# maduc238/simple_distributed_machine_learning

Measured on AMD Instinct MI355X. Metric: samples/sec (whole node), 2-stage MLP on MNIST-shape synthetic, higher is better.
Workload: dtype fp32

## Files before the change

### simple_distributed_machine_learning_amd/csrc/kernels/head_block.h

```cpp
#pragma once

#include <hip/hip_runtime.h>

#include "head_tile.h"
#include "lds_dma.h"

namespace sdml {
namespace hblk {

typedef float hb_f32x16 __attribute__((ext_vector_type(16)));
typedef float hb_f32x4 __attribute__((ext_vector_type(4)));
typedef _Float16 hb_f16x8 __attribute__((ext_vector_type(8)));
typedef _Float16 hb_f16x4 __attribute__((ext_vector_type(4)));
typedef short hb_s16x4 __attribute__((ext_vector_type(4)));
typedef float hb_f32x2 __attribute__((ext_vector_type(2)));
typedef _Float16 hb_f16x2 __attribute__((ext_vector_type(2)));
typedef unsigned hb_u32x2 __attribute__((ext_vector_type(2)));

constexpr int ROWS = 256, HID = 128, NW = 8, NT = 512;
constexpr int PLANE_B = HID * ROWS * 2;
constexpr int DLT_OFF = 2 * PLANE_B;
constexpr int DLT_PLANE_B = 16 * ROWS * 2;
constexpr int RED_OFF = DLT_OFF + 2 * DLT_PLANE_B;
constexpr int RED_FLOATS = 168;
// ... 59 lines not shown
  hb_f32x4 w2c;
  headtile::f32x4m b;
  int tg[2];
};
template <int C>
__device__ __forceinline__ void load_operands(const Args& a, int m0, int M, int wave, int lane, Operands& o) {
  const int r = lane & 15, g = lane >> 4;
  o.w2c = reinterpret_cast<const hb_f32x4*>(a.w2)[min(wave * 64 + lane, C * HID / 4 - 1)];
#pragma unroll
  for (int v = 0; v < 4; ++v) o.b[v] = a.b2[min(4 * g + v, C - 1)];
#pragma unroll
  for (int it = 0; it < 2; ++it)
    o.tg[it] = reinterpret_cast<const int*>(a.target)[2 * (size_t)min(m0 + 16 * (wave + NW * it) + r, M - 1)];
}

struct NoOp {
  __device__ void operator()() const {}
};
template <int C, class Prep, class Hook, class PostB1 = NoOp>
__device__ __forceinline__ void block_head(Prep&& prep, unsigned char* smem, const Args& a, const Operands& ops, int m0,
                                           int M, int wave, int lane, Hook&& hook, long long* stamp,
                                           PostB1&& post_b1 = PostB1{}) {
  static_assert(C >= 2 && C <= 16 && C % 2 == 0, "one 16-class tile; dl stored by class pairs");
  auto st = [&](int k) {
    if (stamp && lane == 0) stamp[k] = (long long)__builtin_amdgcn_s_memtime();
  };
  float* red = reinterpret_cast<float*>(smem + RED_OFF);
  const int wm = wave & 3, wn = wave >> 2, h2 = lane >> 5, r32 = lane & 31;
  const int r = lane & 15, g = lane >> 4;
  const int tid = wave * 64 + lane;
  headtile::f32x4m bv;
#pragma unroll
  for (int v = 0; v < 4; ++v) bv[v] = (4 * g + v) < C ? ops.b[v] : 0.f;
  const int tg[2] = {ops.tg[0], ops.tg[1]};

  hb_f32x16 y[2][2];
  prep(y);
  float hm = 0.f;
#pragma unroll
  for (int i = 0; i < 2; ++i)
#pragma unroll
    for (int j = 0; j < 2; ++j)
#pragma unroll
      for (int q = 0; q < 16; ++q) hm = fmaxf(hm, fabsf(y[i][j][q]));
  hm = wv::max64(hm);
  const float wc = fmaxf(fmaxf(fabsf(ops.w2c[0]), fabsf(ops.w2c[1])), fmaxf(fabsf(ops.w2c[2]), fabsf(ops.w2c[3])));
  const float wmw = wv::max64(wc);
  if (lane == 0) {
    red[wave] = hm;
    red[160 + wave] = wmw;
  }
  __syncthreads();
  st(17);
  post_b1();
  float bm = red[0], wm2 = red[160];
#pragma unroll
  for (int w = 1; w < NW; ++w) {
    bm = fmaxf(bm, red[w]);
    wm2 = fmaxf(wm2, red[160 + w]);
// ... 1 lines not shown
  const int Eh = bexp(bm), Ew = bexp(wm2), Ed = bexp(a.loss_scale);
  const float sh = p2(14 - Eh), sw = p2(14 - Ew), sd = p2(14 - Ed);
  const hb_f32x2 sh2 = {sh, sh}, sd2 = {sd, sd};
  {
    const bool ok = tid < C * HID / 4;
    const hb_f32x2 sw2 = {sw, sw};
    const hb_f32x2 x01 = hb_f32x2{ok ? ops.w2c[0] : 0.f, ok ? ops.w2c[1] : 0.f} * sw2;
    const hb_f32x2 x23 = hb_f32x2{ok ? ops.w2c[2] : 0.f, ok ? ops.w2c[3] : 0.f} * sw2;
    const hb_f16x2 h01 = __builtin_convertvector(x01, hb_f16x2), h23 = __builtin_convertvector(x23, hb_f16x2);
    const hb_f16x2 l01 = lo_pair(h01, x01), l23 = lo_pair(h23, x23);
    unsigned char* dst = smem + W2_OFF + (tid >> 5) * W2PP + 8 * (tid & 31);
    *reinterpret_cast<hb_f16x4*>(dst) = hb_f16x4{h01[0], h01[1], h23[0], h23[1]};
    *reinterpret_cast<hb_f16x4*>(dst + W2PL) = hb_f16x4{l01[0], l01[1], l23[0], l23[1]};
  }

  const int ib0 = hid_base(64 * wn + r32, 16 * wm + h2), ib1 = hid_base(64 * wn + 32 + r32, 16 * wm + h2);
#pragma unroll
  for (int i = 0; i < 2; ++i)
#pragma unroll
    for (int j = 0; j < 2; ++j) {
#pragma unroll
      for (int rq = 0; rq < 4; ++rq) {
        const hb_f32x2 x01 = hb_f32x2{y[i][j][4 * rq], y[i][j][4 * rq + 1]} * sh2;
        const hb_f32x2 x23 = hb_f32x2{y[i][j][4 * rq + 2], y[i][j][4 * rq + 3]} * sh2;
        const hb_f16x2 h01 = __builtin_convertvector(x01, hb_f16x2), h23 = __builtin_convertvector(x23, hb_f16x2);
        const hb_f16x4 hi = {h01[0], h01[1], h23[0], h23[1]};
        const hb_f16x2 l01 = lo_pair(h01, x01), l23 = lo_pair(h23, x23);
        const hb_f16x4 lo = {l01[0], l01[1], l23[0], l23[1]};
        const int o = (j ? ib1 : ib0) ^ (8 * (8 * i + 2 * rq));
        *reinterpret_cast<hb_f16x4*>(smem + o) = hi;
        *reinterpret_cast<hb_f16x4*>(smem + HPL + o) = lo;
      }
    }
  __syncthreads();
  st(18);
  hb_f16x8 wp[4][2];
#pragma unroll
  for (int kk = 0; kk < 4; ++kk)
#pragma unroll
    for (int p = 0; p < 2; ++p)
      wp[kk][p] = *reinterpret_cast<const hb_f16x8*>(smem + W2_OFF + p * W2PL + r * W2PP + 2 * (32 * kk + 8 * g));

  headtile::TileAcc acc;
  acc.zero();
  const float zsc = p2(Eh - 14) * p2(Ew - 14);
  hb_f32x4 dbs = {0.f, 0.f, 0.f, 0.f};
  const int lb0 = hoff(0, 8 * g + (r >> 2), 4 * wave + (r & 3)), lb1 = hoff(0, 8 * g + 4 + (r >> 2), 4 * wave + (r & 3));
  const __amdgpu_buffer_rsrc_t dlr = dma_rsrc(a.dl, (unsigned)((size_t)M * C * 4));
// ... 119 lines not shown
```

### simple_distributed_machine_learning_amd/csrc/kernels/mlp_u8.hip

```cpp
#include <hip/hip_runtime.h>

#include <algorithm>
#include <cstdlib>
#include <type_traits>

#include "head_block.h"
#include "head_reduce.h"
#include "head_tile.h"
#include "lds_dma.h"
#include "kernels.h"
#include "mma_prims.h"
#include "sgd_rule.h"
#include "wave_ops.h"
#include "u8_planes.h"

namespace sdml {
namespace {

typedef unsigned u32x4 __attribute__((ext_vector_type(4)));
typedef _Float16 f16x2 __attribute__((ext_vector_type(2)));

constexpr int FBN = 128;
constexpr int FBK = 64;
constexpr int NS = 2;
constexpr int NSUB = FBK / 16;
constexpr int NPL = kU8FwdPlanes;
constexpr int B_PLANE = FBN * FBK * 2;
constexpr int XCH = FBK / 16;
constexpr int WCH = FBK / 8;
static_assert(FBK == 32 || FBK == 64, "swizzles below are written for 32- and 64-deep K-steps");

template <int WMT, int NWR = 4, int NSG = NS>
struct Geo {
  static constexpr int THREADS = 128 * NWR;
  static constexpr int WAVES = THREADS / 64;
  static constexpr int BM = NWR * 32 * WMT;
  static constexpr int A_BYTES = BM * FBK;
  static constexpr int STAGE = A_BYTES + NPL * B_PLANE;
  static constexpr int GLDS_X = A_BYTES / 1024 / WAVES;
  static constexpr int GLDS_W = NPL * B_PLANE / 1024 / WAVES;
  static constexpr int GLDS_PER_STAGE = GLDS_X + GLDS_W;
  static_assert(GLDS_X * 1024 * WAVES == A_BYTES && GLDS_W * 1024 * WAVES == NPL * B_PLANE, "DMA split");
  static constexpr int EPR = WAVES * 64 * 64 * 4 <= 128 * 1024 ? 64 : 32;
  static constexpr int SMEM = std::max(NSG * STAGE, WAVES * EPR * 64 * 4);
  static_assert(SMEM <= 160 * 1024, "LDS");
};

__device__ __forceinline__ int xpos(int r, int c) { return c ^ (XCH == 2 ? (r >> 3) & 1 : (r >> 2) & 3); }
__device__ __forceinline__ int wpos(int r, int c) { return c ^ (WCH == 4 ? (r >> 2) & 3 : (r >> 1) & 7); }

template <int N>
__device__ __forceinline__ void wait_vmcnt() {
  asm volatile("s_waitcnt vmcnt(%0)" ::"n"(N) : "memory");
}

__device__ __forceinline__ f16x2 h2_of(unsigned v, unsigned sel) {
  const unsigned t = __builtin_amdgcn_perm(0x64646464u, v, sel);
  return __builtin_bit_cast(f16x2, t) - f16x2{(_Float16)1024.f, (_Float16)1024.f};
}
__device__ __forceinline__ f16x8 widen8h(unsigned lo, unsigned hi) {
  const f16x2 a = h2_of(lo, 0x04010400u), b = h2_of(lo, 0x04030402u);
  const f16x2 c = h2_of(hi, 0x04010400u), d = h2_of(hi, 0x04030402u);
  return f16x8{a[0], a[1], b[0], b[1], c[0], c[1], d[0], d[1]};
}

__device__ __forceinline__ f32x16 mfma(f16x8 a, f16x8 b, f32x16 c) {
  return __builtin_amdgcn_mfma_f32_32x32x16_f16(a, b, c, 0, 0, 0);
}

struct FwdParams {
  const unsigned char* X;
  const u16* Wp;
  const float* bias;
  float* C;
  int M, N, K, Kp, ldx, ldc;
  float scale;
  int relu;
  int prio;
  unsigned* mask;
  float* wmax;
  U8HeadArgs head;
  int pf_stride;
// ... 34 lines not shown
  constexpr int WROWS = 1024 / (2 * FBK);
  constexpr int WINST = FBN / WROWS;
  const size_t plane = (size_t)p.N * p.Kp;
#pragma unroll
  for (int u = 0; u < G::GLDS_W; ++u) {
    if (G::GLDS_X + u < U0 || G::GLDS_X + u >= U1) continue;
    const int q = wave + G::WAVES * u;
    const int pl = q / WINST;
    const int row = WROWS * (q % WINST) + lane / WCH;
    const int ch = wpos(row, lane % WCH);
    bdma16(rw, (unsigned)(2 * (pl * plane + (size_t)(n0 + row) * p.Kp + k0 + 8 * ch)), st + G::A_BYTES + 1024 * q);
  }
}

template <int C, int NWR>
__device__ __forceinline__ void fused_head_epilogue(const FwdParams& p, const f32x16 (&acc)[2][2], unsigned char* smem,
                                                    int m0, int wave, int lane, int wm, int wn,
                                                    const hblk::Operands& ops, const float (&bv1)[2], long long* stamp,
                                                    int hb);
template <int C>
__device__ __forceinline__ void fused_head_prefetch(const FwdParams& p, int m0, int wave, int lane, int wn,
                                                    hblk::Operands& ops, float (&bv1)[2]);

template <int MODE, int WMT, int TAIL, int NWR, int HEADC = 0, int NSK = NS, int DMAS = 0>
__global__ void __launch_bounds__(128 * NWR, NWR == 2 ? 2 : 1) u8_fwd_kernel(FwdParams p) {
  constexpr int NS = NSK;
  using G = Geo<WMT, NWR, NSK>;
  static_assert(HEADC == 0 || ((WMT == 2 || WMT == 4) && NWR == 4), "the fused head epilogue: 8 waves of 64 x 64");
  constexpr bool HALVES = HEADC > 0 && WMT == 4;
  auto tile_row = [](int i) { return HALVES ? 32 * (i & 1) + 256 * (i >> 1) : 32 * i; };
  static_assert(HEADC == 0 || G::SMEM <= hblk::LDS_BYTES, "the prefetch scratch KiB sits past the ring and the head");
  constexpr int STAGE = G::STAGE, GLDS_PER_STAGE = G::GLDS_PER_STAGE;
  constexpr int SMEM_BYTES = HEADC ? std::max(G::SMEM, hblk::LDS_BYTES) + 1024 : G::SMEM;
  __shared__ __attribute__((aligned(16))) unsigned char smem[SMEM_BYTES];
  const int m0 = blockIdx.x * G::BM, n0 = blockIdx.y * FBN;
  const int lane = threadIdx.x & 63;
  const int wave = __builtin_amdgcn_readfirstlane(threadIdx.x >> 6);
  const int wm = wave % NWR, wn = wave / NWR;
  if (p.prio && wave >= G::WAVES / 2) __builtin_amdgcn_s_setprio(1);
  const int h = lane >> 5, r32 = lane & 31;
  U8_STAMP(0, __builtin_amdgcn_s_memrealtime);
  U8_STAMP(1, __builtin_amdgcn_s_memtime);
  hblk::Operands hops;
  float hb1[2];

  f32x16 acc[WMT][2];
#pragma unroll
  for (int i = 0; i < WMT; ++i)
#pragma unroll
    for (int j = 0; j < 2; ++j) acc[i][j] = f32x16{};

  int aoff[XCH / 2], boff[NSUB];
  {
    const int row = (HALVES ? wm * 64 : wm * 32 * WMT) + r32;
#pragma unroll
    for (int c = 0; c < XCH / 2; ++c) aoff[c] = row * FBK + 16 * xpos(row, (XCH / 2) * h + c);
  }
  {
    const int row = wn * 64 + r32;
#pragma unroll
    for (int s = 0; s < NSUB; ++s) boff[s] = G::A_BYTES + row * (2 * FBK) + 16 * wpos(row, NSUB * h + s);
  }

  auto load_a = [&](const unsigned char* st, int s2, u32x4 (&ar)[WMT]) {
#pragma unroll
    for (int i = 0; i < WMT; ++i) {
      if constexpr (MODE == 3) ar[i] = u32x4{(unsigned)aoff[s2], 1u, 2u, 3u};
      else ar[i] = *reinterpret_cast<const u32x4*>(st + aoff[s2] + FBK * tile_row(i));
    }
  };
  auto load_b = [&](const unsigned char* st, int s, f16x8 (&b)[2][NPL]) {
#pragma unroll
    for (int j = 0; j < 2; ++j)
#pragma unroll
      for (int pl = 0; pl < NPL; ++pl) {
        if constexpr (MODE == 3) b[j][pl] = __builtin_bit_cast(f16x8, bf16x8{(short)boff[s], (short)pl, (short)j, 2, 3, 4, 5, 6});
        else b[j][pl] = *reinterpret_cast<const f16x8*>(st + boff[s] + 64 * FBK * j + pl * B_PLANE);
      }
  };
  auto compute = [&](int s, const u32x4 (&ar)[WMT], const f16x8 (&b)[2][NPL]) {
#pragma unroll
    for (int i = 0; i < WMT; ++i) {
      const u32x4 v = ar[i];
      f16x8 a;
      if constexpr (MODE == 5) a = __builtin_bit_cast(f16x8, v);
      else a = (s & 1) ? widen8h(v[2], v[3]) : widen8h(v[0], v[1]);
#pragma unroll
      for (int j = 0; j < 2; ++j)
#pragma unroll
        for (int pl = NPL - 1; pl >= 0; --pl) acc[i][j] = mfma(a, b[j][pl], acc[i][j]);
    }
  };
  constexpr int DMA_AT = MODE == 8 ? 0 : (MODE == 9 ? 1 : -1);
  static_assert(DMAS == 0 || (NSK == 2 && DMA_AT < 0 && MODE != 11 && GLDS_PER_STAGE == 6),
                "spread DMA: the 2-stage production loop, 6 pieces per wave");
  constexpr bool PIPE = MODE == 11;
  auto kstep = [&](const unsigned char* st, auto ns_c, auto&& dma, auto&& dma_part) {
    constexpr int NS_ = decltype(ns_c)::value;
    if constexpr (MODE == 1) return;
    if constexpr (PIPE) {
      u32x4 ar[2][WMT];
      f16x8 b[2][2][NPL];
      load_a(st, 0, ar[0]);
      load_b(st, 0, b[0]);
      dma();
#pragma unroll
      for (int s = 0; s < NS_; ++s) {
        if (s + 1 < NS_) {
          if ((s + 1) % 2 == 0) load_a(st, (s + 1) >> 1, ar[((s + 1) >> 1) & 1]);
          load_b(st, s + 1, b[(s + 1) & 1]);
        }
        __builtin_amdgcn_sched_barrier(0);
        compute(s, ar[(s >> 1) & 1], b[s & 1]);
        __builtin_amdgcn_sched_barrier(0);
      }
    } else if constexpr (DMAS == 2) {
      u32x4 ar[2][WMT];
      f16x8 b[2][2][NPL];
      load_a(st, 0, ar[0]);
      load_b(st, 0, b[0]);
#pragma unroll
      for (int s = 0; s < NS_; ++s) {
        if (s + 1 < NS_) {
          if ((s + 1) % 2 == 0) load_a(st, (s + 1) >> 1, ar[((s + 1) >> 1) & 1]);
          load_b(st, s + 1, b[(s + 1) & 1]);
        }
        compute(s, ar[(s >> 1) & 1], b[s & 1]);
        dma_part(s);
      }
    } else {
      u32x4 ar[WMT];
      f16x8 b[2][NPL];
#pragma unroll
      for (int s = 0; s < NS_; ++s) {
        if (s % 2 == 0) load_a(st, s >> 1, ar);
        load_b(st, s, b);
        compute(s, ar, b);
        if (s == DMA_AT) dma();
        if constexpr (DMAS == 1) dma_part(s);
      }
    }
  };

  const int nk = p.Kp / FBK;
#pragma unroll
  for (int t = 0; t < NS - 1; ++t)
    if (t < nk) issue_stage<WMT, NWR>(p, smem + t * STAGE, m0, n0, t * FBK, wave, lane);
  auto sync_step = [&](int t, auto issue_c) {
    const int ahead = min(NS - 2, nk - 1 - t);
    if constexpr (NS >= 4) {
      if (ahead >= 2) wait_vmcnt<2 * GLDS_PER_STAGE>();
      else if (ahead == 1) wait_vmcnt<GLDS_PER_STAGE>();
      else wait_vmcnt<0>();
    } else if constexpr (NS == 3) {
// ... 29 lines not shown
        },
        [&](int sub) {
          if (sub == 0) issue_stage<WMT, NWR, 0, 2>(p, nxt, m0, n0, k1, wave, lane);
          else if (sub == 1) issue_stage<WMT, NWR, 2, 4>(p, nxt, m0, n0, k1, wave, lane);
          else if (sub == 2) issue_stage<WMT, NWR, 4, 1 << 20>(p, nxt, m0, n0, k1, wave, lane);
        });
  }
  {
    sync_step(nk - 1, std::integral_constant<bool, (NS > 2)>{});
    kstep(smem + ((nk - 1) % NS) * STAGE, std::integral_constant<int, TAIL>{}, no_dma, no_dma_part);
  }
  U8_STAMP(15, __builtin_amdgcn_s_memtime);
  if constexpr (MODE == 10) {
    float keep = 0.f;
#pragma unroll
    for (int i = 0; i < WMT; ++i)
#pragma unroll
      for (int j = 0; j < 2; ++j)
#pragma unroll
        for (int r = 0; r < 16; ++r) keep += acc[i][j][r];
    if (keep == 12345.f && lane == 99) p.stamps[0] = 1;
    return;
  }

  if constexpr (HEADC > 0) {
    long long* stp = MODE == 7 ? p.stamps + ((size_t)blockIdx.x * G::WAVES + wave) * U8_NSTAMP : nullptr;
    if constexpr (!HALVES) {
      fused_head_epilogue<HEADC, NWR>(p, acc, smem, m0, wave, lane, wm, wn, hops, hb1, stp, (int)blockIdx.x);
    } else {
      typedef const f32x16 Half[2][2];
      fused_head_epilogue<HEADC, NWR>(p, *reinterpret_cast<Half*>(&acc[0][0]), smem, m0, wave, lane, wm, wn, hops, hb1,
                                      stp, 2 * (int)blockIdx.x);
      if (m0 + hblk::ROWS < p.M) {
        __syncthreads();
        fused_head_prefetch<HEADC>(p, m0 + hblk::ROWS, wave, lane, wn, hops, hb1);
        fused_head_epilogue<HEADC, NWR>(p, *reinterpret_cast<Half*>(&acc[2][0]), smem, m0 + hblk::ROWS, wave, lane, wm,
                                        wn, hops, hb1, nullptr, 2 * (int)blockIdx.x + 1);
      }
    }
    U8_STAMP(22, __builtin_amdgcn_s_memtime);
    U8_STAMP(U8_NSTAMP - 1, __builtin_amdgcn_s_memrealtime);
    return;
  }
  __syncthreads();
  constexpr int EPR = G::EPR, NI2 = EPR / 32;
  float* T = reinterpret_cast<float*>(smem) + wave * EPR * 64;
  float bv[2];
#pragma unroll
  for (int j = 0; j < 2; ++j) bv[j] = p.bias ? p.bias[n0 + wn * 64 + 32 * j + r32] : 0.f;
  float vmax = 0.f;
#pragma unroll
  for (int ip = 0; ip < WMT / NI2; ++ip) {
    asm volatile("s_waitcnt lgkmcnt(0)" ::: "memory");
#pragma unroll
    for (int j = 0; j < 2; ++j)
#pragma unroll
      for (int i2 = 0; i2 < NI2; ++i2)
#pragma unroll
        for (int r = 0; r < 16; ++r) {
          float y = acc[NI2 * ip + i2][j][r] * p.scale + bv[j];
          if (p.relu) y = fmaxf(y, 0.f);
          T[(32 * i2 + (r & 3) + 8 * (r >> 2) + 4 * h) * 64 + 32 * j + r32] = y;
        }
    asm volatile("s_waitcnt lgkmcnt(0)" ::: "memory");
    __builtin_amdgcn_wave_barrier();
#pragma unroll
    for (int q = 0; q < EPR / 4; ++q) {
      const int rr = 4 * q + (lane >> 4);
      const int row = m0 + wm * 32 * WMT + EPR * ip + rr;
      const f32x4 v = *reinterpret_cast<const f32x4*>(T + rr * 64 + 4 * (lane & 15));
      if constexpr (MODE == 6) {
        if (v[0] == 12345.f && row < 0) *reinterpret_cast<f32x4*>(p.C) = v;
      } else if (row < p.M) {
        *reinterpret_cast<f32x4*>(p.C + (size_t)row * p.ldc + n0 + wn * 64 + 4 * (lane & 15)) = v;
        vmax = fmaxf(fmaxf(vmax, fmaxf(fabsf(v[0]), fabsf(v[1]))), fmaxf(fabsf(v[2]), fabsf(v[3])));
      }
      if (p.mask) {
        unsigned w = ((v[0] > 0.f ? 1u : 0u) | (v[1] > 0.f ? 2u : 0u) | (v[2] > 0.f ? 4u : 0u) |
                      (v[3] > 0.f ? 8u : 0u)) << (4 * (lane & 7));
        w |= __shfl_xor(w, 1);
        w |= __shfl_xor(w, 2);
        w |= __shfl_xor(w, 4);
        if ((lane & 7) == 0 && row < p.M)
          p.mask[(size_t)row * (p.N / 32) + (n0 + wn * 64) / 32 + ((lane & 15) >> 3)] = w;
      }
    }
  }
  if (p.wmax) {
    for (int off = 32; off > 0; off >>= 1) vmax = fmaxf(vmax, __shfl_xor(vmax, off));
    if (lane == 0) p.wmax[((size_t)blockIdx.y * gridDim.x + blockIdx.x) * G::WAVES + wave] = vmax;
  }
}

template <int Q>
__device__ __forceinline__ void mask_words(const f32x16 (&y)[2][2], int (&mw)[2]) {
  if constexpr (Q < 64) {
    constexpr int i = Q >> 5, j = (Q >> 4) & 1, r = Q & 15, rw = 32 * i + 8 * (r >> 2);
    const unsigned long long b0 = __ballot(y[i][j][r] > 0.f), b1 = __ballot(y[i][j][r + 1] > 0.f);
    const unsigned long long b2 = __ballot(y[i][j][r + 2] > 0.f), b3 = __ballot(y[i][j][r + 3] > 0.f);
    asm("s_nop 4\n\t"
        "v_writelane_b32 %0, %1, %9\n\tv_writelane_b32 %0, %2, %10\n\t"
        "v_writelane_b32 %0, %3, %11\n\tv_writelane_b32 %0, %4, %12\n\t"
        "v_writelane_b32 %0, %5, %13\n\tv_writelane_b32 %0, %6, %14\n\t"
        "v_writelane_b32 %0, %7, %15\n\tv_writelane_b32 %0, %8, %16"
        : "+v"(mw[j])
        : "s"((unsigned)b0), "s"((unsigned)(b0 >> 32)), "s"((unsigned)b1), "s"((unsigned)(b1 >> 32)),
          "s"((unsigned)b2), "s"((unsigned)(b2 >> 32)), "s"((unsigned)b3), "s"((unsigned)(b3 >> 32)),
          "i"(rw), "i"(rw + 4), "i"(rw + 1), "i"(rw + 5), "i"(rw + 2), "i"(rw + 6), "i"(rw + 3), "i"(rw + 7));
    mask_words<Q + 4>(y, mw);
  }
}

template <int C>
__device__ __forceinline__ hblk::Args fused_head_args(const FwdParams& p, int hb) {
  const U8HeadArgs& hd = p.head;
  hblk::Args a;
  a.w2 = hd.w2;
  a.b2 = hd.b2;
  a.target = hd.target;
  a.loss_scale = hd.loss_scale;
  a.train = true;
  a.dl = hd.dl;
  a.part = hd.part + (size_t)hb * (C * 128 + C + 2);
  a.bound = hd.bound + hb;
  return a;
}

template <int C>
__device__ __forceinline__ void fused_head_prefetch(const FwdParams& p, int m0, int wave, int lane, int wn,
                                                    hblk::Operands& ops, float (&bv1)[2]) {
  hblk::load_operands<C>(fused_head_args<C>(p, 0), m0, p.M, wave, lane, ops);
#pragma unroll
  for (int j = 0; j < 2; ++j) bv1[j] = p.bias[wn * 64 + 32 * j + (lane & 31)];
}

template <int C, int NWR>
__device__ __forceinline__ void fused_head_epilogue(const FwdParams& p, const f32x16 (&acc)[2][2], unsigned char* smem,
                                                    int m0, int wave, int lane, int wm, int wn,
                                                    const hblk::Operands& ops, const float (&bv1)[2], long long* stamp,
                                                    int hb) {
  static_assert(NWR == 4, "head_block.h: 8 waves of 64 x 64, 256 rows");
  const U8HeadArgs& hd = p.head;
  const int h2 = lane >> 5;
  if (stamp && lane == 0) stamp[16] = (long long)__builtin_amdgcn_s_memtime();
  const hblk::Args a = fused_head_args<C>(p, hb);
  auto prep = [&](hblk::hb_f32x16 (&y)[2][2]) {
    const hblk::hb_f32x2 sc2 = {p.scale, p.scale};
#pragma unroll
    for (int i = 0; i < 2; ++i)
#pragma unroll
      for (int j = 0; j < 2; ++j) {
        const hblk::hb_f32x2 b2 = {bv1[j], bv1[j]};
#pragma unroll
        for (int r = 0; r < 16; r += 2) {
          const hblk::hb_f32x2 v = __builtin_elementwise_fma(hblk::hb_f32x2{acc[i][j][r], acc[i][j][r + 1]}, sc2, b2);
          y[i][j][r] = fmaxf(v[0], 0.f);
          y[i][j][r + 1] = fmaxf(v[1], 0.f);
        }
      }
    if (m0 + hblk::ROWS > p.M) {
#pragma unroll
      for (int i = 0; i < 2; ++i)
#pragma unroll
        for (int j = 0; j < 2; ++j)
#pragma unroll
          for (int r = 0; r < 16; ++r)
            if (m0 + wm * 64 + 32 * i + (r & 3) + 8 * (r >> 2) + 4 * h2 >= p.M) y[i][j][r] = 0.f;
    }
    int mw[2] = {0, 0};
    mask_words<0>(y, mw);
    const int row = m0 + wm * 64 + lane;
    if (row < p.M) *reinterpret_cast<uint2*>(hd.mask + (size_t)row * 4 + 2 * wn) = uint2{(unsigned)mw[0], (unsigned)mw[1]};
  };
  const bool pf = p.pf_stride > 0 && (int)blockIdx.x + p.pf_stride < (int)gridDim.x;
  auto post_b1 = [&]() {
    if (pf) {
      const int m1 = ((int)blockIdx.x + p.pf_stride) * hblk::ROWS;
      const dma_i32x4 rx = dma_rsrc4(p.X, (unsigned)((size_t)p.M * p.ldx));
#pragma unroll
      for (int u = 0; u < 2; ++u) {
        const int row = 16 * (wave + 8 * u) + (lane >> 2);
        const unsigned voff = (unsigned)((size_t)min(m1 + row, p.M - 1) * p.ldx + 16 * (lane & 3));
        bdma16_asm(rx, voff, 0u, smem + hblk::LDS_BYTES);
      }
    }
  };
  hblk::block_head<C>(prep, smem, a, ops, m0, p.M, wave, lane, [](int, int, bool, const float (&)[4]) {}, stamp,
                      post_b1);
  if (pf) asm volatile("s_waitcnt vmcnt(0)" ::: "memory");
}

__global__ void __launch_bounds__(256) split_planes_pad_kernel(const float* __restrict__ w, u16* __restrict__ out,
                                                               int N, int K, int Kp) {
  const int64_t i = (int64_t)blockIdx.x * 256 + threadIdx.x;
  const int64_t n = (int64_t)N * Kp;
  if (i >= n) return;
  const int r = (int)(i / Kp), k = (int)(i % Kp);
  const float x = k < K ? w[(size_t)r * K + k] : 0.f;
  u16 hi, lo;
  u8_fwd_planes_of(x, hi, lo);
  out[i] = hi;
  out[n + i] = lo;
}
// ... 854 lines not shown
  int dev = 0;
  if (hipGetDevice(&dev) != hipSuccess || dev < 0 || dev >= 64) return nullptr;
  if (!words[dev]) {
    hipStreamCaptureStatus cs = hipStreamCaptureStatusNone;
    if (hipStreamIsCapturing(stream, &cs) != hipSuccess || cs != hipStreamCaptureStatusNone) return nullptr;
    void* w = nullptr;
    if (hipMalloc(&w, 4096 * sizeof(unsigned)) != hipSuccess) return nullptr;
    if (hipMemset(w, 0, 4096 * sizeof(unsigned)) != hipSuccess) return nullptr;
    words[dev] = static_cast<unsigned*>(w);
  }
  return words[dev];
}

static int tail_substeps(int K) {
  const int v = K - ((K + FBK - 1) / FBK - 1) * FBK;
  if (v > FBK / 2 - 8) return NSUB;
  if (NSUB == 4 && v > 16) return 3;
  if (NSUB == 4 && v > 8) return 2;
  return 1;
}

int u8_fwd_kpad(int K) { return (K + FBK - 1) / FBK * FBK; }

bool u8_fwd_supported(int M, int N, int K, int ldx, const void* X) {
  return M >= 256 && N % FBN == 0 && K >= 16 && K % 16 == 0 && ldx % 16 == 0 &&
         (reinterpret_cast<uintptr_t>(X) & 15) == 0 && (int64_t)M * ldx < (int64_t(1) << 31);
}

bool u8_wgrad_supported(int M, int N, int K, int ldx, const void* X, const void* dz) {
  return K == GKC && N % GHN == 0 && M % GBK == 0 && M >= GBK && ldx % 16 == 0 &&
         (reinterpret_cast<uintptr_t>(X) & 15) == 0 && (reinterpret_cast<uintptr_t>(dz) & 15) == 0 &&
         (int64_t)M * ldx < (int64_t(1) << 31);
}

// ... 168 lines not shown
  }();
#else
  constexpr int mode = 0;
#endif
  bool w16;
  int wmt, bm;
  u8_fwd_geometry(M, w16, wmt, bm);
  const dim3 grid((M + bm - 1) / bm, N / FBN);
  const int tail = tail_substeps(K);
#define FWD_LAUNCH(MD, W, T, R) \
  hipLaunchKernelGGL((u8_fwd_kernel<MD, W, T, R>), grid, dim3(Geo<W, R>::THREADS), 0, stream, p)
#define FWD_TAILS(W, R)                          \
  do {                                           \
    switch (tail) {                              \
      case 1: FWD_LAUNCH(0, W, 1, R); break;     \
      case 2: FWD_LAUNCH(0, W, 2, R); break;     \
      case 3: FWD_LAUNCH(0, W, 3, R); break;     \
      default: FWD_LAUNCH(0, W, NSUB, R);        \
    }                                            \
  } while (0)
#define FWD_MODE(MD)                                \
  do {                                              \
    if (w16) FWD_LAUNCH(MD, 2, NSUB, 8);            \
    else if (wmt == 4) FWD_LAUNCH(MD, 4, NSUB, 4);  \
    else FWD_LAUNCH(MD, 2, NSUB, 4);                \
  } while (0)
#ifdef SDML_KERNEL_EXPERIMENTS
  if (mode == 1) FWD_MODE(1);
  else if (mode == 2) FWD_MODE(2);
  else if (mode == 3) FWD_MODE(3);
  else if (mode == 4) FWD_MODE(4);
  else if (mode == 5) FWD_MODE(5);
// ... 100 lines not shown
      case 4: FHM(4); break;
      case 5: FHM(5); break;
      case 8: FHM(8); break;
      case 9: FHM(9); break;
      case 10: FHM(10); break;
      case 11: FHM(11); break;
      default: abort();
    }
#undef FHM
    return;
  }
  if (g_u8_stamps && head.C == 10) {
    p.stamps = g_u8_stamps;
    switch (tail) {
      case 1: hipLaunchKernelGGL((u8_fwd_kernel<7, 2, 1, 4, 10>), grid, dim3(512), 0, stream, p); break;
      case 2: hipLaunchKernelGGL((u8_fwd_kernel<7, 2, 2, 4, 10>), grid, dim3(512), 0, stream, p); break;
      case 3: hipLaunchKernelGGL((u8_fwd_kernel<7, 2, 3, 4, 10>), grid, dim3(512), 0, stream, p); break;
      default: hipLaunchKernelGGL((u8_fwd_kernel<7, 2, NSUB, 4, 10>), grid, dim3(512), 0, stream, p);
    }
    return;
  }
#endif
  const dim3 grid512((M + Geo<4, 4>::BM - 1) / Geo<4, 4>::BM, 1);
  if (rows512) p.pf_stride = 0;
#define FH_LAUNCH(T, CC)                                                                                    \
  do {                                                                                                      \
    if (rows512) hipLaunchKernelGGL((u8_fwd_kernel<0, 4, T, 4, CC>), grid512, dim3(512), 0, stream, p);       \
    else if (spread == 2) hipLaunchKernelGGL((u8_fwd_kernel<0, 2, T, 4, CC, NS, 2>), grid, dim3(512), 0, stream, p); \
    else if (spread) hipLaunchKernelGGL((u8_fwd_kernel<0, 2, T, 4, CC, NS, 1>), grid, dim3(512), 0, stream, p); \
    else hipLaunchKernelGGL((u8_fwd_kernel<0, 2, T, 4, CC>), grid, dim3(512), 0, stream, p);               \
  } while (0)
#define FH_LAUNCH3(T) hipLaunchKernelGGL((u8_fwd_kernel<0, 2, T, 4, 10, 3>), grid, dim3(512), 0, stream, p)
#define FH_TAILS(CC)                      \
  do {                                    \
    switch (tail) {                       \
      case 1: FH_LAUNCH(1, CC); break;    \
      case 2: FH_LAUNCH(2, CC); break;    \
      case 3: FH_LAUNCH(3, CC); break;    \
      default: FH_LAUNCH(NSUB, CC);       \
    }                                     \
  } while (0)
  if (head.C == 10 && knob(KNOB_U8_FH_STAGES) == 3) {
    switch (tail) {
      case 1: FH_LAUNCH3(1); break;
      case 2: FH_LAUNCH3(2); break;
      case 3: FH_LAUNCH3(3); break;
      default: FH_LAUNCH3(NSUB);
    }
    return;
  }
  switch (head.C) {
    case 10: FH_TAILS(10); break;
    case 2: FH_TAILS(2); break;
    case 16: FH_TAILS(16); break;
    default: abort();
  }
#undef FH_TAILS
#undef FH_LAUNCH3
#undef FH_LAUNCH
}

// ... 2 lines not shown
```

Baseline: 993.5 million.

## Switch u8 forward GEMM from 32x32x16 to 16x16x32 MFMA tiles

Replaces the 32x32x16 f16 MFMA in the u8 forward kernel with the 16x16x32 variant. This reworks the accumulator layout (4x4 tiles of f32x4), the A/B LDS swizzles, the load/widen/compute pipeline, the tail sub-step logic and the epilogue. The fused head path gets a Map16 lane mapping and a rewritten ReLU mask packing to match the new accumulator layout. The aim is a shorter MFMA latency and better operand reuse per K-step. The cost is more LDS B loads per column tile and a reworked, riskier swizzle and mask mapping.

```diff
diff --git a/simple_distributed_machine_learning_amd/csrc/kernels/head_block.h b/simple_distributed_machine_learning_amd/csrc/kernels/head_block.h
--- a/simple_distributed_machine_learning_amd/csrc/kernels/head_block.h
+++ b/simple_distributed_machine_learning_amd/csrc/kernels/head_block.h
@@ -1,6 +1,8 @@
 #pragma once
 
 #include <hip/hip_runtime.h>
+
+#include <type_traits>
 
 #include "head_tile.h"
 #include "lds_dma.h"
@@ -97,13 +99,18 @@
     o.tg[it] = reinterpret_cast<const int*>(a.target)[2 * (size_t)min(m0 + 16 * (wave + NW * it) + r, M - 1)];
 }
 
+struct Map32 {};
+struct Map16 {};
+
 struct NoOp {
   __device__ void operator()() const {}
 };
-template <int C, class Prep, class Hook, class PostB1 = NoOp>
+template <int C, class Prep, class Hook, class PostB1 = NoOp, class Map = Map32>
 __device__ __forceinline__ void block_head(Prep&& prep, unsigned char* smem, const Args& a, const Operands& ops, int m0,
                                            int M, int wave, int lane, Hook&& hook, long long* stamp,
-                                           PostB1&& post_b1 = PostB1{}) {
+                                           PostB1&& post_b1 = PostB1{}, Map = Map{}) {
+  constexpr bool M16 = std::is_same<Map, Map16>::value;
+  constexpr int YA = M16 ? 4 : 2, YV = M16 ? 4 : 16;
   static_assert(C >= 2 && C <= 16 && C % 2 == 0, "one 16-class tile; dl stored by class pairs");
   auto st = [&](int k) {
     if (stamp && lane == 0) stamp[k] = (long long)__builtin_amdgcn_s_memtime();
@@ -117,15 +124,15 @@
   for (int v = 0; v < 4; ++v) bv[v] = (4 * g + v) < C ? ops.b[v] : 0.f;
   const int tg[2] = {ops.tg[0], ops.tg[1]};
 
-  hb_f32x16 y[2][2];
+  typename std::conditional<M16, hb_f32x4, hb_f32x16>::type y[YA][YA];
   prep(y);
   float hm = 0.f;
 #pragma unroll
-  for (int i = 0; i < 2; ++i)
-#pragma unroll
-    for (int j = 0; j < 2; ++j)
-#pragma unroll
-      for (int q = 0; q < 16; ++q) hm = fmaxf(hm, fabsf(y[i][j][q]));
+  for (int i = 0; i < YA; ++i)
+#pragma unroll
+    for (int j = 0; j < YA; ++j)
+#pragma unroll
+      for (int q = 0; q < YV; ++q) hm = fmaxf(hm, fabsf(y[i][j][q]));
   hm = wv::max64(hm);
   const float wc = fmaxf(fmaxf(fabsf(ops.w2c[0]), fabsf(ops.w2c[1])), fmaxf(fabsf(ops.w2c[2]), fabsf(ops.w2c[3])));
   const float wmw = wv::max64(wc);
@@ -157,24 +164,36 @@
     *reinterpret_cast<hb_f16x4*>(dst + W2PL) = hb_f16x4{l01[0], l01[1], l23[0], l23[1]};
   }
 
-  const int ib0 = hid_base(64 * wn + r32, 16 * wm + h2), ib1 = hid_base(64 * wn + 32 + r32, 16 * wm + h2);
-#pragma unroll
-  for (int i = 0; i < 2; ++i)
-#pragma unroll
-    for (int j = 0; j < 2; ++j) {
-#pragma unroll
-      for (int rq = 0; rq < 4; ++rq) {
-        const hb_f32x2 x01 = hb_f32x2{y[i][j][4 * rq], y[i][j][4 * rq + 1]} * sh2;
-        const hb_f32x2 x23 = hb_f32x2{y[i][j][4 * rq + 2], y[i][j][4 * rq + 3]} * sh2;
-        const hb_f16x2 h01 = __builtin_convertvector(x01, hb_f16x2), h23 = __builtin_convertvector(x23, hb_f16x2);
-        const hb_f16x4 hi = {h01[0], h01[1], h23[0], h23[1]};
-        const hb_f16x2 l01 = lo_pair(h01, x01), l23 = lo_pair(h23, x23);
-        const hb_f16x4 lo = {l01[0], l01[1], l23[0], l23[1]};
-        const int o = (j ? ib1 : ib0) ^ (8 * (8 * i + 2 * rq));
-        *reinterpret_cast<hb_f16x4*>(smem + o) = hi;
-        *reinterpret_cast<hb_f16x4*>(smem + HPL + o) = lo;
+  auto put = [&](float v0, float v1, float v2, float v3, int o) {
+    const hb_f32x2 x01 = hb_f32x2{v0, v1} * sh2;
+    const hb_f32x2 x23 = hb_f32x2{v2, v3} * sh2;
+    const hb_f16x2 h01 = __builtin_convertvector(x01, hb_f16x2), h23 = __builtin_convertvector(x23, hb_f16x2);
+    const hb_f16x4 hi = {h01[0], h01[1], h23[0], h23[1]};
+    const hb_f16x2 l01 = lo_pair(h01, x01), l23 = lo_pair(h23, x23);
+    const hb_f16x4 lo = {l01[0], l01[1], l23[0], l23[1]};
+    *reinterpret_cast<hb_f16x4*>(smem + o) = hi;
+    *reinterpret_cast<hb_f16x4*>(smem + HPL + o) = lo;
+  };
+  if constexpr (M16) {
+#pragma unroll
+    for (int c = 0; c < 4; ++c) {
+      const int ib = hoff(0, 64 * wn + 16 * c + r, 16 * wm + g);
+#pragma unroll
+      for (int t = 0; t < 4; ++t) put(y[t][c][0], y[t][c][1], y[t][c][2], y[t][c][3], ib ^ (8 * (4 * t)));
+    }
+  } else {
+    const int ib0 = hid_base(64 * wn + r32, 16 * wm + h2), ib1 = hid_base(64 * wn + 32 + r32, 16 * wm + h2);
+#pragma unroll
+    for (int i = 0; i < 2; ++i)
+#pragma unroll
+      for (int j = 0; j < 2; ++j) {
+#pragma unroll
+        for (int rq = 0; rq < 4; ++rq) {
+          const int o = (j ? ib1 : ib0) ^ (8 * (8 * i + 2 * rq));
+          put(y[i][j][4 * rq], y[i][j][4 * rq + 1], y[i][j][4 * rq + 2], y[i][j][4 * rq + 3], o);
+        }
       }
-    }
+  }
   __syncthreads();
   st(18);
   hb_f16x8 wp[4][2];
diff --git a/simple_distributed_machine_learning_amd/csrc/kernels/mlp_u8.hip b/simple_distributed_machine_learning_amd/csrc/kernels/mlp_u8.hip
--- a/simple_distributed_machine_learning_amd/csrc/kernels/mlp_u8.hip
+++ b/simple_distributed_machine_learning_amd/csrc/kernels/mlp_u8.hip
@@ -23,12 +23,13 @@
 constexpr int FBN = 128;
 constexpr int FBK = 64;
 constexpr int NS = 2;
-constexpr int NSUB = FBK / 16;
+constexpr int NSUB = FBK / 32;
 constexpr int NPL = kU8FwdPlanes;
 constexpr int B_PLANE = FBN * FBK * 2;
 constexpr int XCH = FBK / 16;
 constexpr int WCH = FBK / 8;
-static_assert(FBK == 32 || FBK == 64, "swizzles below are written for 32- and 64-deep K-steps");
+static_assert(FBK == 64, "the lane map (k-group g = lane >> 4 <-> pixel chunk g) and the swizzles below are written for "
+                         "64-deep K-steps");
 
 template <int WMT, int NWR = 4, int NSG = NS>
 struct Geo {
@@ -46,8 +47,8 @@
   static_assert(SMEM <= 160 * 1024, "LDS");
 };
 
-__device__ __forceinline__ int xpos(int r, int c) { return c ^ (XCH == 2 ? (r >> 3) & 1 : (r >> 2) & 3); }
-__device__ __forceinline__ int wpos(int r, int c) { return c ^ (WCH == 4 ? (r >> 2) & 3 : (r >> 1) & 7); }
+__device__ __forceinline__ int xpos(int r, int c) { return c ^ ((-(r >> 2)) & 3); }
+__device__ __forceinline__ int wpos(int r, int c) { return c ^ ((r & 6) | (((r >> 2) ^ (r >> 3) ^ 1) & 1)); }
 
 template <int N>
 __device__ __forceinline__ void wait_vmcnt() {
@@ -66,6 +67,9 @@
 
 __device__ __forceinline__ f32x16 mfma(f16x8 a, f16x8 b, f32x16 c) {
   return __builtin_amdgcn_mfma_f32_32x32x16_f16(a, b, c, 0, 0, 0);
+}
+__device__ __forceinline__ f32x4 mfma16(f16x8 a, f16x8 b, f32x4 c) {
+  return __builtin_amdgcn_mfma_f32_16x16x32_f16(a, b, c, 0, 0, 0);
 }
 
 struct FwdParams {
@@ -130,13 +134,13 @@
 }
 
 template <int C, int NWR>
-__device__ __forceinline__ void fused_head_epilogue(const FwdParams& p, const f32x16 (&acc)[2][2], unsigned char* smem,
+__device__ __forceinline__ void fused_head_epilogue(const FwdParams& p, const f32x4 (&acc)[4][4], unsigned char* smem,
                                                     int m0, int wave, int lane, int wm, int wn,
-                                                    const hblk::Operands& ops, const float (&bv1)[2], long long* stamp,
+                                                    const hblk::Operands& ops, const float (&bv1)[4], long long* stamp,
                                                     int hb);
 template <int C>
 __device__ __forceinline__ void fused_head_prefetch(const FwdParams& p, int m0, int wave, int lane, int wn,
-                                                    hblk::Operands& ops, float (&bv1)[2]);
+                                                    hblk::Operands& ops, float (&bv1)[4]);
 
 template <int MODE, int WMT, int TAIL, int NWR, int HEADC = 0, int NSK = NS, int DMAS = 0>
 __global__ void __launch_bounds__(128 * NWR, NWR == 2 ? 2 : 1) u8_fwd_kernel(FwdParams p) {
@@ -144,7 +148,11 @@
   using G = Geo<WMT, NWR, NSK>;
   static_assert(HEADC == 0 || ((WMT == 2 || WMT == 4) && NWR == 4), "the fused head epilogue: 8 waves of 64 x 64");
   constexpr bool HALVES = HEADC > 0 && WMT == 4;
-  auto tile_row = [](int i) { return HALVES ? 32 * (i & 1) + 256 * (i >> 1) : 32 * i; };
+  constexpr int RT = 2 * WMT, CT = 4;
+  auto tile_row = [](int t) {
+    const int i = t >> 1;
+    return (HALVES ? 32 * (i & 1) + 256 * (i >> 1) : 32 * i) + 16 * (t & 1);
+  };
   static_assert(HEADC == 0 || G::SMEM <= hblk::LDS_BYTES, "the prefetch scratch KiB sits past the ring and the head");
   constexpr int STAGE = G::STAGE, GLDS_PER_STAGE = G::GLDS_PER_STAGE;
   constexpr int SMEM_BYTES = HEADC ? std::max(G::SMEM, hblk::LDS_BYTES) + 1024 : G::SMEM;
@@ -154,58 +162,56 @@
   const int wave = __builtin_amdgcn_readfirstlane(threadIdx.x >> 6);
   const int wm = wave % NWR, wn = wave / NWR;
   if (p.prio && wave >= G::WAVES / 2) __builtin_amdgcn_s_setprio(1);
-  const int h = lane >> 5, r32 = lane & 31;
+  const int g16 = lane >> 4, r16 = lane & 15;
   U8_STAMP(0, __builtin_amdgcn_s_memrealtime);
   U8_STAMP(1, __builtin_amdgcn_s_memtime);
   hblk::Operands hops;
-  float hb1[2];
-
-  f32x16 acc[WMT][2];
-#pragma unroll
-  for (int i = 0; i < WMT; ++i)
-#pragma unroll
-    for (int j = 0; j < 2; ++j) acc[i][j] = f32x16{};
-
-  int aoff[XCH / 2], boff[NSUB];
+  float hb1[CT];
+
+  f32x4 acc[RT][CT];
+#pragma unroll
+  for (int t = 0; t < RT; ++t)
+#pragma unroll
+    for (int c = 0; c < CT; ++c) acc[t][c] = f32x4{};
+
+  int aoff, boff[NSUB];
   {
-    const int row = (HALVES ? wm * 64 : wm * 32 * WMT) + r32;
-#pragma unroll
-    for (int c = 0; c < XCH / 2; ++c) aoff[c] = row * FBK + 16 * xpos(row, (XCH / 2) * h + c);
+    const int row = (HALVES ? wm * 64 : wm * 32 * WMT) + r16;
+    aoff = row * FBK + 16 * xpos(row, g16);
   }
   {
-    const int row = wn * 64 + r32;
-#pragma unroll
-    for (int s = 0; s < NSUB; ++s) boff[s] = G::A_BYTES + row * (2 * FBK) + 16 * wpos(row, NSUB * h + s);
-  }
-
-  auto load_a = [&](const unsigned char* st, int s2, u32x4 (&ar)[WMT]) {
-#pragma unroll
-    for (int i = 0; i < WMT; ++i) {
-      if constexpr (MODE == 3) ar[i] = u32x4{(unsigned)aoff[s2], 1u, 2u, 3u};
-      else ar[i] = *reinterpret_cast<const u32x4*>(st + aoff[s2] + FBK * tile_row(i));
-    }
-  };
-  auto load_b = [&](const unsigned char* st, int s, f16x8 (&b)[2][NPL]) {
-#pragma unroll
-    for (int j = 0; j < 2; ++j)
-#pragma unroll
-      for (int pl = 0; pl < NPL; ++pl) {
-        if constexpr (MODE == 3) b[j][pl] = __builtin_bit_cast(f16x8, bf16x8{(short)boff[s], (short)pl, (short)j, 2, 3, 4, 5, 6});
-        else b[j][pl] = *reinterpret_cast<const f16x8*>(st + boff[s] + 64 * FBK * j + pl * B_PLANE);
-      }
-  };
-  auto compute = [&](int s, const u32x4 (&ar)[WMT], const f16x8 (&b)[2][NPL]) {
-#pragma unroll
-    for (int i = 0; i < WMT; ++i) {
-      const u32x4 v = ar[i];
-      f16x8 a;
-      if constexpr (MODE == 5) a = __builtin_bit_cast(f16x8, v);
-      else a = (s & 1) ? widen8h(v[2], v[3]) : widen8h(v[0], v[1]);
-#pragma unroll
-      for (int j = 0; j < 2; ++j)
-#pragma unroll
-        for (int pl = NPL - 1; pl >= 0; --pl) acc[i][j] = mfma(a, b[j][pl], acc[i][j]);
-    }
+    const int row = wn * 64 + r16;
+#pragma unroll
+    for (int s = 0; s < NSUB; ++s) boff[s] = G::A_BYTES + row * (2 * FBK) + 16 * wpos(row, NSUB * g16 + s);
+  }
+
+  auto load_a = [&](const unsigned char* st, u32x4 (&ar)[RT]) {
+#pragma unroll
+    for (int t = 0; t < RT; ++t) {
+      if constexpr (MODE == 3) ar[t] = u32x4{(unsigned)aoff, 1u, 2u, 3u};
+      else ar[t] = *reinterpret_cast<const u32x4*>(st + aoff + FBK * tile_row(t));
+    }
+  };
+  auto load_b = [&](const unsigned char* st, int s, int c, f16x8 (&b)[NPL]) {
+#pragma unroll
+    for (int pl = 0; pl < NPL; ++pl) {
+      if constexpr (MODE == 3) b[pl] = __builtin_bit_cast(f16x8, bf16x8{(short)boff[s], (short)pl, (short)c, 2, 3, 4, 5, 6});
+      else b[pl] = *reinterpret_cast<const f16x8*>(st + boff[s] + 16 * (2 * FBK) * c + pl * B_PLANE);
+    }
+  };
+  auto widen = [&](int s, const u32x4 (&ar)[RT], f16x8 (&a)[RT]) {
+#pragma unroll
+    for (int t = 0; t < RT; ++t) {
+      const u32x4 v = ar[t];
+      if constexpr (MODE == 5) a[t] = __builtin_bit_cast(f16x8, v);
+      else a[t] = s ? widen8h(v[2], v[3]) : widen8h(v[0], v[1]);
+    }
+  };
+  auto compute = [&](int c, const f16x8 (&a)[RT], const f16x8 (&b)[NPL]) {
+#pragma unroll
+    for (int pl = NPL - 1; pl >= 0; --pl)
+#pragma unroll
+      for (int t = 0; t < RT; ++t) acc[t][c] = mfma16(a[t], b[pl], acc[t][c]);
   };
   constexpr int DMA_AT = MODE == 8 ? 0 : (MODE == 9 ? 1 : -1);
   static_assert(DMAS == 0 || (NSK == 2 && DMA_AT < 0 && MODE != 11 && GLDS_PER_STAGE == 6),
@@ -214,46 +220,40 @@
   auto kstep = [&](const unsigned char* st, auto ns_c, auto&& dma, auto&& dma_part) {
     constexpr int NS_ = decltype(ns_c)::value;
     if constexpr (MODE == 1) return;
-    if constexpr (PIPE) {
-      u32x4 ar[2][WMT];
-      f16x8 b[2][2][NPL];
-      load_a(st, 0, ar[0]);
-      load_b(st, 0, b[0]);
-      dma();
+    u32x4 ar[RT];
+    f16x8 a[RT];
+    if constexpr (PIPE || DMAS == 2) {
+      f16x8 b[2][NPL];
+      load_a(st, ar);
+      load_b(st, 0, 0, b[0]);
+      if constexpr (PIPE) dma();
+#pragma unroll
+      for (int q = 0; q < CT * NS_; ++q) {
+        if (q % CT == 0) widen(q / CT, ar, a);
+        if (q + 1 < CT * NS_) load_b(st, (q + 1) / CT, (q + 1) % CT, b[(q + 1) & 1]);
+        if constexpr (PIPE) __builtin_amdgcn_sched_barrier(0);
+        compute(q % CT, a, b[q & 1]);
+        if constexpr (PIPE) __builtin_amdgcn_sched_barrier(0);
+        if constexpr (DMAS == 2) {
+          if (q & 1) dma_part(q >> 1);
+        }
+      }
+    } else {
+      f16x8 b[NPL];
+      load_a(st, ar);
 #pragma unroll
       for (int s = 0; s < NS_; ++s) {
-        if (s + 1 < NS_) {
-          if ((s + 1) % 2 == 0) load_a(st, (s + 1) >> 1, ar[((s + 1) >> 1) & 1]);
-          load_b(st, s + 1, b[(s + 1) & 1]);
+        widen(s, ar, a);
+#pragma unroll
+        for (int c = 0; c < CT; ++c) {
+          load_b(st, s, c, b);
+          compute(c, a, b);
+          if constexpr (NWR == 8) __builtin_amdgcn_sched_barrier(0);
+          if constexpr (DMAS == 1) {
+            if (c & 1) dma_part(2 * s + (c >> 1));
+          }
         }
-        __builtin_amdgcn_sched_barrier(0);
-        compute(s, ar[(s >> 1) & 1], b[s & 1]);
-        __builtin_amdgcn_sched_barrier(0);
-      }
-    } else if constexpr (DMAS == 2) {
-      u32x4 ar[2][WMT];
-      f16x8 b[2][2][NPL];
-      load_a(st, 0, ar[0]);
-      load_b(st, 0, b[0]);
-#pragma unroll
-      for (int s = 0; s < NS_; ++s) {
-        if (s + 1 < NS_) {
-          if ((s + 1) % 2 == 0) load_a(st, (s + 1) >> 1, ar[((s + 1) >> 1) & 1]);
-          load_b(st, s + 1, b[(s + 1) & 1]);
-        }
-        compute(s, ar[(s >> 1) & 1], b[s & 1]);
-        dma_part(s);
-      }
-    } else {
-      u32x4 ar[WMT];
-      f16x8 b[2][NPL];
-#pragma unroll
-      for (int s = 0; s < NS_; ++s) {
-        if (s % 2 == 0) load_a(st, s >> 1, ar);
-        load_b(st, s, b);
-        compute(s, ar, b);
         if (s == DMA_AT) dma();
-        if constexpr (DMAS == 1) dma_part(s);
       }
     }
   };
@@ -313,11 +313,11 @@
   if constexpr (MODE == 10) {
     float keep = 0.f;
 #pragma unroll
-    for (int i = 0; i < WMT; ++i)
-#pragma unroll
-      for (int j = 0; j < 2; ++j)
-#pragma unroll
-        for (int r = 0; r < 16; ++r) keep += acc[i][j][r];
+    for (int t = 0; t < RT; ++t)
+#pragma unroll
+      for (int c = 0; c < CT; ++c)
+#pragma unroll
+        for (int v = 0; v < 4; ++v) keep += acc[t][c][v];
     if (keep == 12345.f && lane == 99) p.stamps[0] = 1;
     return;
   }
@@ -327,13 +327,13 @@
     if constexpr (!HALVES) {
       fused_head_epilogue<HEADC, NWR>(p, acc, smem, m0, wave, lane, wm, wn, hops, hb1, stp, (int)blockIdx.x);
     } else {
-      typedef const f32x16 Half[2][2];
+      typedef const f32x4 Half[4][4];
       fused_head_epilogue<HEADC, NWR>(p, *reinterpret_cast<Half*>(&acc[0][0]), smem, m0, wave, lane, wm, wn, hops, hb1,
                                       stp, 2 * (int)blockIdx.x);
       if (m0 + hblk::ROWS < p.M) {
         __syncthreads();
         fused_head_prefetch<HEADC>(p, m0 + hblk::ROWS, wave, lane, wn, hops, hb1);
-        fused_head_epilogue<HEADC, NWR>(p, *reinterpret_cast<Half*>(&acc[2][0]), smem, m0 + hblk::ROWS, wave, lane, wm,
+        fused_head_epilogue<HEADC, NWR>(p, *reinterpret_cast<Half*>(&acc[4][0]), smem, m0 + hblk::ROWS, wave, lane, wm,
                                         wn, hops, hb1, nullptr, 2 * (int)blockIdx.x + 1);
       }
     }
@@ -342,24 +342,24 @@
     return;
   }
   __syncthreads();
-  constexpr int EPR = G::EPR, NI2 = EPR / 32;
+  constexpr int EPR = G::EPR, NI2 = EPR / 16;
   float* T = reinterpret_cast<float*>(smem) + wave * EPR * 64;
-  float bv[2];
-#pragma unroll
-  for (int j = 0; j < 2; ++j) bv[j] = p.bias ? p.bias[n0 + wn * 64 + 32 * j + r32] : 0.f;
+  float bv[CT];
+#pragma unroll
+  for (int c = 0; c < CT; ++c) bv[c] = p.bias ? p.bias[n0 + wn * 64 + 16 * c + r16] : 0.f;
   float vmax = 0.f;
 #pragma unroll
-  for (int ip = 0; ip < WMT / NI2; ++ip) {
+  for (int ip = 0; ip < RT / NI2; ++ip) {
     asm volatile("s_waitcnt lgkmcnt(0)" ::: "memory");
 #pragma unroll
-    for (int j = 0; j < 2; ++j)
+    for (int c = 0; c < CT; ++c)
 #pragma unroll
       for (int i2 = 0; i2 < NI2; ++i2)
 #pragma unroll
-        for (int r = 0; r < 16; ++r) {
-          float y = acc[NI2 * ip + i2][j][r] * p.scale + bv[j];
+        for (int v = 0; v < 4; ++v) {
+          float y = acc[NI2 * ip + i2][c][v] * p.scale + bv[c];
           if (p.relu) y = fmaxf(y, 0.f);
-          T[(32 * i2 + (r & 3) + 8 * (r >> 2) + 4 * h) * 64 + 32 * j + r32] = y;
+          T[(16 * i2 + 4 * g16 + v) * 64 + ((16 * c + r16 + 16 * (4 * i2 + g16)) & 63)] = y;
         }
     asm volatile("s_waitcnt lgkmcnt(0)" ::: "memory");
     __builtin_amdgcn_wave_barrier();
@@ -367,7 +367,7 @@
     for (int q = 0; q < EPR / 4; ++q) {
       const int rr = 4 * q + (lane >> 4);
       const int row = m0 + wm * 32 * WMT + EPR * ip + rr;
-      const f32x4 v = *reinterpret_cast<const f32x4*>(T + rr * 64 + 4 * (lane & 15));
+      const f32x4 v = *reinterpret_cast<const f32x4*>(T + rr * 64 + ((4 * (lane & 15) + 16 * q) & 63));
       if constexpr (MODE == 6) {
         if (v[0] == 12345.f && row < 0) *reinterpret_cast<f32x4*>(p.C) = v;
       } else if (row < p.M) {
@@ -391,22 +391,43 @@
   }
 }
 
-template <int Q>
-__device__ __forceinline__ void mask_words(const f32x16 (&y)[2][2], int (&mw)[2]) {
-  if constexpr (Q < 64) {
-    constexpr int i = Q >> 5, j = (Q >> 4) & 1, r = Q & 15, rw = 32 * i + 8 * (r >> 2);
-    const unsigned long long b0 = __ballot(y[i][j][r] > 0.f), b1 = __ballot(y[i][j][r + 1] > 0.f);
-    const unsigned long long b2 = __ballot(y[i][j][r + 2] > 0.f), b3 = __ballot(y[i][j][r + 3] > 0.f);
-    asm("s_nop 4\n\t"
-        "v_writelane_b32 %0, %1, %9\n\tv_writelane_b32 %0, %2, %10\n\t"
-        "v_writelane_b32 %0, %3, %11\n\tv_writelane_b32 %0, %4, %12\n\t"
-        "v_writelane_b32 %0, %5, %13\n\tv_writelane_b32 %0, %6, %14\n\t"
-        "v_writelane_b32 %0, %7, %15\n\tv_writelane_b32 %0, %8, %16"
-        : "+v"(mw[j])
-        : "s"((unsigned)b0), "s"((unsigned)(b0 >> 32)), "s"((unsigned)b1), "s"((unsigned)(b1 >> 32)),
-          "s"((unsigned)b2), "s"((unsigned)(b2 >> 32)), "s"((unsigned)b3), "s"((unsigned)(b3 >> 32)),
-          "i"(rw), "i"(rw + 4), "i"(rw + 1), "i"(rw + 5), "i"(rw + 2), "i"(rw + 6), "i"(rw + 3), "i"(rw + 7));
-    mask_words<Q + 4>(y, mw);
+typedef unsigned short mw_u16x2 __attribute__((ext_vector_type(2)));
+__device__ __forceinline__ unsigned pack_ll(unsigned a, unsigned b) {
+  return __builtin_bit_cast(unsigned, mw_u16x2{(unsigned short)a, (unsigned short)b});
+}
+__device__ __forceinline__ unsigned pack_hh(unsigned a, unsigned b) {
+  return __builtin_bit_cast(unsigned, mw_u16x2{(unsigned short)(a >> 16), (unsigned short)(b >> 16)});
+}
+template <int t>
+__device__ __forceinline__ void mask_words(const f32x4 (&y)[4][4], int (&mw)[2]) {
+  if constexpr (t < 4) {
+    unsigned long long bl[4][4];
+#pragma unroll
+    for (int v = 0; v < 4; ++v)
+#pragma unroll
+      for (int c = 0; c < 4; ++c) bl[v][c] = __ballot(y[t][c][v] > 0.f);
+    __builtin_amdgcn_sched_barrier(0);
+#pragma unroll
+    for (int v = 0; v < 4; ++v) {
+      unsigned w[2][4];
+#pragma unroll
+      for (int j = 0; j < 2; ++j) {
+        const unsigned long long lo = bl[v][2 * j], hi = bl[v][2 * j + 1];
+        w[j][0] = pack_ll((unsigned)lo, (unsigned)hi);
+        w[j][1] = pack_hh((unsigned)lo, (unsigned)hi);
+        w[j][2] = pack_ll((unsigned)(lo >> 32), (unsigned)(hi >> 32));
+        w[j][3] = pack_hh((unsigned)(lo >> 32), (unsigned)(hi >> 32));
+      }
+      asm("s_nop 4\n\t"
+          "v_writelane_b32 %0, %2, %10\n\tv_writelane_b32 %0, %3, %11\n\t"
+          "v_writelane_b32 %0, %4, %12\n\tv_writelane_b32 %0, %5, %13\n\t"
+          "v_writelane_b32 %1, %6, %10\n\tv_writelane_b32 %1, %7, %11\n\t"
+          "v_writelane_b32 %1, %8, %12\n\tv_writelane_b32 %1, %9, %13"
+          : "+v"(mw[0]), "+v"(mw[1])
+          : "s"(w[0][0]), "s"(w[0][1]), "s"(w[0][2]), "s"(w[0][3]), "s"(w[1][0]), "s"(w[1][1]), "s"(w[1][2]),
+            "s"(w[1][3]), "i"(16 * t + v), "i"(16 * t + 4 + v), "i"(16 * t + 8 + v), "i"(16 * t + 12 + v));
+    }
+    mask_words<t + 1>(y, mw);
   }
 }
 
@@ -427,44 +448,44 @@
 
 template <int C>
 __device__ __forceinline__ void fused_head_prefetch(const FwdParams& p, int m0, int wave, int lane, int wn,
-                                                    hblk::Operands& ops, float (&bv1)[2]) {
+                                                    hblk::Operands& ops, float (&bv1)[4]) {
   hblk::load_operands<C>(fused_head_args<C>(p, 0), m0, p.M, wave, lane, ops);
 #pragma unroll
-  for (int j = 0; j < 2; ++j) bv1[j] = p.bias[wn * 64 + 32 * j + (lane & 31)];
+  for (int c = 0; c < 4; ++c) bv1[c] = p.bias[wn * 64 + 16 * c + (lane & 15)];
 }
 
 template <int C, int NWR>
-__device__ __forceinline__ void fused_head_epilogue(const FwdParams& p, const f32x16 (&acc)[2][2], unsigned char* smem,
+__device__ __forceinline__ void fused_head_epilogue(const FwdParams& p, const f32x4 (&acc)[4][4], unsigned char* smem,
                                                     int m0, int wave, int lane, int wm, int wn,
-                                                    const hblk::Operands& ops, const float (&bv1)[2], long long* stamp,
+                                                    const hblk::Operands& ops, const float (&bv1)[4], long long* stamp,
                                                     int hb) {
   static_assert(NWR == 4, "head_block.h: 8 waves of 64 x 64, 256 rows");
   const U8HeadArgs& hd = p.head;
-  const int h2 = lane >> 5;
+  const int g16 = lane >> 4;
   if (stamp && lane == 0) stamp[16] = (long long)__builtin_amdgcn_s_memtime();
   const hblk::Args a = fused_head_args<C>(p, hb);
-  auto prep = [&](hblk::hb_f32x16 (&y)[2][2]) {
+  auto prep = [&](hblk::hb_f32x4 (&y)[4][4]) {
     const hblk::hb_f32x2 sc2 = {p.scale, p.scale};
 #pragma unroll
-    for (int i = 0; i < 2; ++i)
-#pragma unroll
-      for (int j = 0; j < 2; ++j) {
-        const hblk::hb_f32x2 b2 = {bv1[j], bv1[j]};
-#pragma unroll
-        for (int r = 0; r < 16; r += 2) {
-          const hblk::hb_f32x2 v = __builtin_elementwise_fma(hblk::hb_f32x2{acc[i][j][r], acc[i][j][r + 1]}, sc2, b2);
-          y[i][j][r] = fmaxf(v[0], 0.f);
-          y[i][j][r + 1] = fmaxf(v[1], 0.f);
+    for (int t = 0; t < 4; ++t)
+#pragma unroll
+      for (int c = 0; c < 4; ++c) {
+        const hblk::hb_f32x2 b2 = {bv1[c], bv1[c]};
+#pragma unroll
+        for (int v = 0; v < 4; v += 2) {
+          const hblk::hb_f32x2 x = __builtin_elementwise_fma(hblk::hb_f32x2{acc[t][c][v], acc[t][c][v + 1]}, sc2, b2);
+          y[t][c][v] = fmaxf(x[0], 0.f);
+          y[t][c][v + 1] = fmaxf(x[1], 0.f);
         }
       }
     if (m0 + hblk::ROWS > p.M) {
 #pragma unroll
-      for (int i = 0; i < 2; ++i)
-#pragma unroll
-        for (int j = 0; j < 2; ++j)
-#pragma unroll
-          for (int r = 0; r < 16; ++r)
-            if (m0 + wm * 64 + 32 * i + (r & 3) + 8 * (r >> 2) + 4 * h2 >= p.M) y[i][j][r] = 0.f;
+      for (int t = 0; t < 4; ++t)
+#pragma unroll
+        for (int c = 0; c < 4; ++c)
+#pragma unroll
+          for (int v = 0; v < 4; ++v)
+            if (m0 + wm * 64 + 16 * t + 4 * g16 + v >= p.M) y[t][c][v] = 0.f;
     }
     int mw[2] = {0, 0};
     mask_words<0>(y, mw);
@@ -485,7 +506,7 @@
     }
   };
   hblk::block_head<C>(prep, smem, a, ops, m0, p.M, wave, lane, [](int, int, bool, const float (&)[4]) {}, stamp,
-                      post_b1);
+                      post_b1, hblk::Map16{});
   if (pf) asm volatile("s_waitcnt vmcnt(0)" ::: "memory");
 }
 
@@ -1370,10 +1391,7 @@
 
 static int tail_substeps(int K) {
   const int v = K - ((K + FBK - 1) / FBK - 1) * FBK;
-  if (v > FBK / 2 - 8) return NSUB;
-  if (NSUB == 4 && v > 16) return 3;
-  if (NSUB == 4 && v > 8) return 2;
-  return 1;
+  return v > 8 ? NSUB : 1;
 }
 
 int u8_fwd_kpad(int K) { return (K + FBK - 1) / FBK * FBK; }
@@ -1572,8 +1590,6 @@
   do {                                           \
     switch (tail) {                              \
       case 1: FWD_LAUNCH(0, W, 1, R); break;     \
-      case 2: FWD_LAUNCH(0, W, 2, R); break;     \
-      case 3: FWD_LAUNCH(0, W, 3, R); break;     \
       default: FWD_LAUNCH(0, W, NSUB, R);        \
     }                                            \
   } while (0)
@@ -1704,8 +1720,6 @@
     p.stamps = g_u8_stamps;
     switch (tail) {
       case 1: hipLaunchKernelGGL((u8_fwd_kernel<7, 2, 1, 4, 10>), grid, dim3(512), 0, stream, p); break;
-      case 2: hipLaunchKernelGGL((u8_fwd_kernel<7, 2, 2, 4, 10>), grid, dim3(512), 0, stream, p); break;
-      case 3: hipLaunchKernelGGL((u8_fwd_kernel<7, 2, 3, 4, 10>), grid, dim3(512), 0, stream, p); break;
       default: hipLaunchKernelGGL((u8_fwd_kernel<7, 2, NSUB, 4, 10>), grid, dim3(512), 0, stream, p);
     }
     return;
@@ -1725,16 +1739,12 @@
   do {                                    \
     switch (tail) {                       \
       case 1: FH_LAUNCH(1, CC); break;    \
-      case 2: FH_LAUNCH(2, CC); break;    \
-      case 3: FH_LAUNCH(3, CC); break;    \
       default: FH_LAUNCH(NSUB, CC);       \
     }                                     \
   } while (0)
   if (head.C == 10 && knob(KNOB_U8_FH_STAGES) == 3) {
     switch (tail) {
       case 1: FH_LAUNCH3(1); break;
-      case 2: FH_LAUNCH3(2); break;
-      case 3: FH_LAUNCH3(3); break;
       default: FH_LAUNCH3(NSUB);
     }
     return;
```

Result: faster. 1.009 billion (median of 6 runs) (+1.6%).
